# kianmcevoy/audio_analysis

Measured on AMD Instinct MI355X. Metric: IRs/sec full report (STFT+RT60bands+zplane), 48 kHz 10 s IR, higher is better.
Workload: dtype f64; 1 GPU; metrics-only full report on 256 mono synthetic IRs per GPU per step, 10 s @ 48 kHz (SURVEY.md 8d generator), H2D included: every step uploads its batch from pinned host memory (float32, 492 MB) on a copy stream under the previous step's kernels; 4 distinct batches rotate; batch_per_gpu=256, parallelism=file-sharded dp1, gather=final

## Files before the change

### audio_analysis_amd/csrc/ira_stft4.hip

```cpp
#include <cmath>
#include <cstdlib>

#include "ira_fft_reg.h"
#include "ira_log.h"
#include "ira_stft.h"

namespace {

using ira::brev_bits;
using ira::cplx;
using ira::dft_dif;
using ira::powers16;

typedef cplx<double> cdd;

constexpr int M4 = 4096, F4 = M4 + 1, TL4 = 128;
constexpr int ROW4 = 129;
constexpr int E2N4 = 256;
constexpr int EXC4 = 16 * ROW4;
static_assert(EXC4 >= 8 * E2N4 && EXC4 * 2 >= M4, "exchange buffer too small");

__device__ __forceinline__ float db_of4(double re, double im, double floor_pow, float floor_db,
                                        const ira::LogTabEntry* tab) {
  const double p = fma(re, re, im * im);
  if (!(p > floor_pow)) return floor_db;
  return (float)(3.0102999566398120 * ira::log2_table<4>(p, tab));
}

__device__ __forceinline__ double lin_of4(double re, double im, double floor_pow, float floor_db, double floor_lin32,
                                          const ira::LogTabEntry* tab) {
  const double p = fma(re, re, im * im);
  if (!(p > floor_pow)) return floor_lin32;
  const double db = 3.0102999566398120 * ira::log2_table<4>(p, tab);
  const double t = ((double)(float)db - db) * 0.11512925464970228;
  const double y0 = __builtin_amdgcn_rsq(p);
  double g = p * y0;
  const double h = 0.5 * y0;
  const double r = fma(-h, g, 0.5);
  g = fma(g, r, g);
  return g * fma(t, fma(t, 0.5, 1.0), 1.0);
}

constexpr int TL5 = 256;
constexpr int KF5 = 8;

struct __attribute__((aligned(4))) fpair5 { float a, b; };
struct __attribute__((aligned(8))) dpair5 { double a, b; };

__global__ __launch_bounds__(TL5) __attribute__((amdgpu_waves_per_eu(4, 4))) void stft5_kernel(
    const float* __restrict__ x, const int64_t* __restrict__ off, const int32_t* __restrict__ nframes, int hop,
    const double* __restrict__ window, const cdd* __restrict__ tw, double floor_lin, float floor_db,
    float* __restrict__ out, const int64_t* __restrict__ out_off, const int32_t* __restrict__ frame_sel,
    const int64_t* __restrict__ sel_off, int lb_nbins, int lb_kbase, const int32_t* __restrict__ lb_first,
    const int32_t* __restrict__ lb_count, int kfr, int ablate) {
  __shared__ __attribute__((aligned(16))) cdd ex[EXC4];
  __shared__ double wave_energy[2][TL5 / 64];
  __shared__ ira::LogTabEntry ltab[ira::LOGTAB_N];
  __shared__ int lb_range[2];
  __shared__ int frame_bad;
  unsigned bx, by;
  ira::xcd_remap(bx, by);
  const int seg = (int)by;
  const int col0 = (int)bx * kfr;
  const int T_out = ira::uniform(nframes[seg]);
  if (col0 >= T_out) return;
  const int col1 = T_out - col0 < kfr ? T_out : col0 + kfr;
  int q = threadIdx.x;
  double* exd = reinterpret_cast<double*>(ex);
  ira::build_log_table(ltab, q);
  if (q < 2) lb_range[q] = q == 0 ? F4 : 0;

  const float* xs = x + ira::uniform(off[seg]);
  float* os = out + ira::uniform(out_off[seg]);
  const int32_t* fsel = frame_sel ? frame_sel + ira::uniform(sel_off[seg]) : nullptr;
  const double floor_pow = floor_lin * floor_lin;
  const float qnan32 = __uint_as_float(0x7fc00000u);
  int k_lo = 0, k_hi = 0;
  double floor_lin32 = 0.0;
  __syncthreads();
  if (lb_nbins > 0) {
    int lo = F4, hi = 0;
    for (int bb = q; bb < lb_nbins; bb += TL5) {
      const int c = lb_count[bb];
      if (c > 0) {
        const int f0 = lb_kbase + lb_first[bb];
        lo = f0 < lo ? f0 : lo;
        hi = f0 + c > hi ? f0 + c : hi;
      }
    }
    atomicMin(&lb_range[0], lo);
    atomicMax(&lb_range[1], hi);
    __syncthreads();
    k_lo = ira::uniform(lb_range[0]);
    k_hi = ira::uniform(lb_range[1]);
    floor_lin32 = ira::uniform(exp10((double)floor_db * 0.05));
  }

  for (int col = col0; col < col1; ++col) {
    asm volatile("" : "+v"(q));
    const int k1l = q & 15, n3l = q >> 4;
    const bool lower = q < TL4;
    const int64_t frame = fsel ? (int64_t)ira::uniform(fsel[col]) : (int64_t)col;
    const float* fx = xs + frame * hop;
    int u0 = 0;
    asm volatile("" : "+s"(u0));
    cdd wuni[8];
#pragma unroll
    for (int i = 0; i < 8; ++i) wuni[i] = tw[TL5 * i + u0];

    cdd v[16];
    double energy = 0.0;
    {
      float xa[16], xb[16];
      double wa[16], wb[16];
#pragma unroll
      for (int n1 = 0; n1 < 16; ++n1) {
        const int n = n1 * 256 + q;
        if (IRA_ABL(ablate & 2)) { xa[n1] = (float)(n & 7) * 0.125f; xb[n1] = (float)(q & 3); }
        else { const fpair5 p = *reinterpret_cast<const fpair5*>(fx + 2 * n); xa[n1] = p.a; xb[n1] = p.b; }
        if (IRA_ABL(ablate & 1)) { wa[n1] = 0.5 + 1e-4 * n1; wb[n1] = 0.25; }
        else { const dpair5 w = *reinterpret_cast<const dpair5*>(window + 2 * n); wa[n1] = w.a; wb[n1] = w.b; }
      }
      __builtin_amdgcn_sched_barrier(0);
#pragma unroll
      for (int n1 = 0; n1 < 16; ++n1) {
        v[n1] = {(double)xa[n1] * wa[n1], (double)xb[n1] * wb[n1]};
        energy = fma(v[n1].re, v[n1].re, energy);
        energy = fma(v[n1].im, v[n1].im, energy);
      }
    }

    double* we = wave_energy[col & 1];
    {
      const double wsum = ira::wave_sum(energy);
      if ((q & 63) == 0) we[q >> 6] = wsum;
    }
    __syncthreads();
    const double frame_energy = ira::uniform((we[0] + we[1]) + (we[2] + we[3]));
    const bool quiet = !IRA_ABL(ablate & 256) && frame_energy * (4.0 * (2 * M4)) <= floor_pow;

    bool bad_frame = false;
    if (quiet) {
      if (lb_nbins <= 0) {
        float* fo = os + (int64_t)col * F4;
#pragma unroll
        for (int i = 0; i < 8; ++i) {
          const int k = q + TL5 * i;
          fo[k] = floor_db;
          fo[M4 - k] = floor_db;
        }
        if (q == 0) fo[M4 / 2] = floor_db;
        continue;
      }
      double fl = floor_lin32;
      asm volatile("" : "+s"(fl));
#pragma unroll
      for (int i = 0; i < 8; ++i) {
        const int k = q + TL5 * i;
        if (k >= k_lo && k < k_hi) exd[k] = fl;
        if ((M4 - k) >= k_lo && (M4 - k) < k_hi) exd[M4 - k] = fl;
      }
      if (q == 0 && M4 / 2 >= k_lo && M4 / 2 < k_hi) exd[M4 / 2] = fl;
    } else {
      dft_dif<double, 16>(v);
      ira::twiddle16<double, true>(v, tw[2 * q]);

      cdd b[16];
      if (lower) {
#pragma unroll
        for (int k1 = 0; k1 < 16; ++k1) ex[k1 * ROW4 + q] = v[brev_bits(k1, 4)];
      }
      __syncthreads();
#pragma unroll
      for (int n2 = 0; n2 < 8; ++n2) b[n2] = ex[k1l * ROW4 + n2 * 16 + n3l];
      __syncthreads();
      if (!lower) {
#pragma unroll
        for (int k1 = 0; k1 < 16; ++k1) ex[k1 * ROW4 + (q - TL4)] = v[brev_bits(k1, 4)];
      }
      __syncthreads();
#pragma unroll
      for (int n2 = 0; n2 < 8; ++n2) b[8 + n2] = ex[k1l * ROW4 + n2 * 16 + n3l];
      __syncthreads();

      dft_dif<double, 16>(b);
      ira::twiddle16<double, true>(b, tw[32 * n3l]);
      if (lower) {
#pragma unroll
        for (int k2 = 0; k2 < 16; ++k2) ex[k1l + 16 * k2 + E2N4 * n3l] = b[brev_bits(k2, 4)];
      }
      __syncthreads();
#pragma unroll
      for (int n3 = 0; n3 < 8; ++n3) v[n3] = ex[q + E2N4 * n3];
      __syncthreads();
      if (!lower) {
#pragma unroll
        for (int k2 = 0; k2 < 16; ++k2) ex[k1l + 16 * k2 + E2N4 * (n3l - 8)] = b[brev_bits(k2, 4)];
      }
      __syncthreads();
#pragma unroll
      for (int n3 = 0; n3 < 8; ++n3) v[8 + n3] = ex[q + E2N4 * n3];
      __syncthreads();

      dft_dif<double, 16>(v);

      double zkr[8], zpr[8], zki[8], zpi[8], midr, midi;
#pragma unroll
      for (int j = 0; j < 8; ++j) ex[j * TL5 + q] = v[brev_bits(8 + j, 4)];
      __syncthreads();
      {
        const int partner = (TL5 - q) & (TL5 - 1);
#pragma unroll
        for (int i = 0; i < 8; ++i) {
          const int slot = q == 0 ? 8 - i : 7 - i;
          cdd zp = v[0];
          if (!(q == 0 && i == 0)) zp = ex[slot * TL5 + partner];
          zkr[i] = v[brev_bits(i, 4)].re; zki[i] = v[brev_bits(i, 4)].im;
          zpr[i] = zp.re; zpi[i] = zp.im;
        }
      }
      {
        const cdd mid = ex[0];
        midr = mid.re; midi = mid.im;
      }
      if (q == 0) frame_bad = !((zkr[0] - zkr[0]) + (zki[0] - zki[0]) == 0.0) ? 1 : 0;
      __syncthreads();
      bad_frame = frame_bad != 0;

      const cdd wlane = tw[q];
      if (lb_nbins <= 0) {
        float* fo = os + (int64_t)col * F4;
#pragma unroll
        for (int i = 0; i < 8; ++i) {
          const int k = q + TL5 * i;
          const cdd e = {0.5 * (zkr[i] + zpr[i]), 0.5 * (zki[i] - zpi[i])};
          const cdd d = {0.5 * (zkr[i] - zpr[i]), 0.5 * (zki[i] + zpi[i])};
          const cdd o = {d.im, -d.re};
          const cdd wk = ira::cmul(wlane, wuni[i]);
          const cdd pp = ira::cmul(wk, o);
          fo[k] = bad_frame ? qnan32 : db_of4(e.re + pp.re, e.im + pp.im, floor_pow, floor_db, ltab);
          fo[M4 - k] = bad_frame ? qnan32 : db_of4(e.re - pp.re, e.im - pp.im, floor_pow, floor_db, ltab);
        }
        if (q == 0) fo[M4 / 2] = bad_frame ? qnan32 : db_of4(midr, midi, floor_pow, floor_db, ltab);
        continue;
      }
#pragma unroll
      for (int i = 0; i < 8; ++i) {
        const int k = q + TL5 * i;
        const bool need_a = k >= k_lo && k < k_hi, need_b = (M4 - k) >= k_lo && (M4 - k) < k_hi;
        if (!need_a && !need_b) continue;
        const cdd e = {0.5 * (zkr[i] + zpr[i]), 0.5 * (zki[i] - zpi[i])};
        const cdd d = {0.5 * (zkr[i] - zpr[i]), 0.5 * (zki[i] + zpi[i])};
        const cdd o = {d.im, -d.re};
        const cdd wk = ira::cmul(wlane, wuni[i]);
        const cdd pp = ira::cmul(wk, o);
        if (IRA_ABL(ablate & 4)) {
          if (need_a) exd[k] = e.re + pp.re;
          if (need_b) exd[M4 - k] = e.im - pp.im;
          continue;
        }
        if (need_a) exd[k] = lin_of4(e.re + pp.re, e.im + pp.im, floor_pow, floor_db, floor_lin32, ltab);
        if (need_b) exd[M4 - k] = lin_of4(e.re - pp.re, e.im - pp.im, floor_pow, floor_db, floor_lin32, ltab);
      }
      if (q == 0 && M4 / 2 >= k_lo && M4 / 2 < k_hi) exd[M4 / 2] = lin_of4(midr, midi, floor_pow, floor_db, floor_lin32, ltab);
    }
    __syncthreads();
    for (int bb = q; bb < lb_nbins; bb += TL5) {
      const int c = lb_count[bb];
      float val = qnan32;
      if (c > 0) {
        const double* r = exd + lb_kbase + lb_first[bb];
        double acc = r[0];
        for (int k0 = 1; k0 < c; k0 += 8) {
          double v8[8];
#pragma unroll
          for (int u = 0; u < 8; ++u) v8[u] = (k0 + u < c) ? r[k0 + u] : 0.0;
#pragma unroll
          for (int u = 0; u < 8; ++u)
            if (k0 + u < c) acc += v8[u];
        }
        val = (float)(6.0205999132796239 * ira::log2_table<6>(fmax(acc / (double)c, 1e-30), ltab));
      }
      os[(int64_t)bb * T_out + col] = (bad_frame && c > 0) ? qnan32 : val;
    }
    __syncthreads();
  }
}

}

int32_t ira_stft5_launch(const float* x, const int64_t* off, const int32_t* nframes, int32_t nseg, int32_t max_frames,
                         int32_t hop, const void* window, const void* tw, double floor_db, float* out,
                         const int64_t* out_off, const int32_t* frame_sel, const int64_t* sel_off, int32_t lb_nbins,
                         int32_t lb_kbase, const int32_t* lb_first, const int32_t* lb_count, hipStream_t st) {
  const double floor_lin = std::pow(10.0, floor_db / 20.0);
  int kfr = ira_tune_int("IRA_STFT5_K", KF5);
  if (kfr < 1) kfr = 1;
  dim3 grid((max_frames + kfr - 1) / kfr, nseg);
  stft5_kernel<<<grid, TL5, (size_t)ira_tune_int("IRA_STFT5_LDS_PAD", 0), st>>>(x, off, nframes, hop, static_cast<const double*>(window),
                                     static_cast<const cdd*>(tw), floor_lin, (float)floor_db, out, out_off, frame_sel,
                                     sel_off, lb_nbins, lb_kbase, lb_first, lb_count, kfr, ira_tune_int("IRA_STFT5_ABLATE", 0));
  IRA_RETURN_LAUNCH();
}
```

Measured before the change: 16610 IRs/s.

## Skip whole quiet STFT frame chunks via block-level energy bound

Before the per-frame loop, each block sums the squared input over the span covering all of its frames. It bounds the windowed energy by the peak squared window value, and when the bound is below the floor it writes floor values for every frame and exits early. Quiet frames inside the loop also write cached log-bin floor values straight to output instead of filling LDS and taking the shared reduction path. This adds a cheap pre-pass and extra LDS per block. The bound must be conservative or non-quiet frames could be wrongly floored, which matters most for the decaying tails of IRs.

```diff
diff --git a/audio_analysis_amd/csrc/ira_stft4.hip b/audio_analysis_amd/csrc/ira_stft4.hip
--- a/audio_analysis_amd/csrc/ira_stft4.hip
+++ b/audio_analysis_amd/csrc/ira_stft4.hip
@@ -41,11 +41,27 @@
   return g * fma(t, fma(t, 0.5, 1.0), 1.0);
 }
 
+template <bool CONST>
+__device__ __forceinline__ float logbin_mean_db(const double* r, double cst, int c, const ira::LogTabEntry* tab) {
+  double acc = CONST ? cst : r[0];
+  for (int k0 = 1; k0 < c; k0 += 8) {
+    double v8[8];
+#pragma unroll
+    for (int u = 0; u < 8; ++u) v8[u] = (k0 + u < c) ? (CONST ? cst : r[k0 + u]) : 0.0;
+#pragma unroll
+    for (int u = 0; u < 8; ++u)
+      if (k0 + u < c) acc += v8[u];
+  }
+  return (float)(6.0205999132796239 * ira::log2_table<6>(fmax(acc / (double)c, 1e-30), tab));
+}
+
 constexpr int TL5 = 256;
 constexpr int KF5 = 8;
 
 struct __attribute__((aligned(4))) fpair5 { float a, b; };
 struct __attribute__((aligned(8))) dpair5 { double a, b; };
+typedef float fquad5 __attribute__((ext_vector_type(4), aligned(4)));
+constexpr int64_t SPAN5_MAX = 2 * (2 * M4);
 
 __global__ __launch_bounds__(TL5) __attribute__((amdgpu_waves_per_eu(4, 4))) void stft5_kernel(
     const float* __restrict__ x, const int64_t* __restrict__ off, const int32_t* __restrict__ nframes, int hop,
@@ -55,6 +71,9 @@
     const int32_t* __restrict__ lb_count, int kfr, int ablate) {
   __shared__ __attribute__((aligned(16))) cdd ex[EXC4];
   __shared__ double wave_energy[2][TL5 / 64];
+  __shared__ double chunk_energy[TL5 / 64];
+  __shared__ unsigned long long chunk_wmax[TL5 / 64];
+  __shared__ float quiet_val[TL5];
   __shared__ ira::LogTabEntry ltab[ira::LOGTAB_N];
   __shared__ int lb_range[2];
   __shared__ int frame_bad;
@@ -95,6 +114,79 @@
     k_hi = ira::uniform(lb_range[1]);
     floor_lin32 = ira::uniform(exp10((double)floor_db * 0.05));
   }
+  auto quiet_bin = [&](int bb, double fl) -> float {
+    const int c = lb_count[bb];
+    return c > 0 ? logbin_mean_db<true>(nullptr, fl, c, ltab) : qnan32;
+  };
+
+  if (!IRA_ABL(ablate & (256 | 512)) && fsel == nullptr && (int64_t)(col1 - col0 - 1) * hop + 2 * M4 <= SPAN5_MAX) {
+    const int nfr = col1 - col0;
+    const int span = (nfr - 1) * hop + 2 * M4;
+    const float* cx = xs + (int64_t)col0 * hop;
+    const int n4 = span >> 2;
+    double s = 0.0;
+    for (int i0 = 0; i0 < n4; i0 += 4 * TL5) {
+      fquad5 p[4];
+#pragma unroll
+      for (int u = 0; u < 4; ++u) {
+        const int i = i0 + u * TL5 + q;
+        p[u] = i < n4 ? *reinterpret_cast<const fquad5*>(cx + 4 * i) : fquad5{0.0f, 0.0f, 0.0f, 0.0f};
+      }
+#pragma unroll
+      for (int u = 0; u < 4; ++u) {
+        s = fma((double)p[u].x, (double)p[u].x, s);
+        s = fma((double)p[u].y, (double)p[u].y, s);
+        s = fma((double)p[u].z, (double)p[u].z, s);
+        s = fma((double)p[u].w, (double)p[u].w, s);
+      }
+    }
+    if (q < (span & 3)) {
+      const double t = (double)cx[4 * n4 + q];
+      s = fma(t, t, s);
+    }
+    {
+      const double wsum = ira::wave_sum(s);
+      if ((q & 63) == 0) chunk_energy[q >> 6] = wsum;
+    }
+    __syncthreads();
+    const double scaled = ira::uniform((chunk_energy[0] + chunk_energy[1]) + (chunk_energy[2] + chunk_energy[3])) * (4.0 * (2 * M4));
+    if (scaled <= 16.0 * floor_pow) {
+      unsigned long long wb = 0;
+#pragma unroll
+      for (int j = 0; j < 2 * M4 / (2 * TL5); ++j) {
+        const dpair5 w = *reinterpret_cast<const dpair5*>(window + 2 * (j * TL5 + q));
+        const unsigned long long ba = (unsigned long long)__double_as_longlong(w.a * w.a) & 0x7fffffffffffffffull;
+        const unsigned long long bb = (unsigned long long)__double_as_longlong(w.b * w.b) & 0x7fffffffffffffffull;
+        wb = ba > wb ? ba : wb;
+        wb = bb > wb ? bb : wb;
+      }
+#pragma unroll
+      for (int o = 32; o > 0; o >>= 1) {
+        const unsigned long long other = __shfl_xor(wb, o, 64);
+        wb = other > wb ? other : wb;
+      }
+      if ((q & 63) == 0) chunk_wmax[q >> 6] = wb;
+      __syncthreads();
+      unsigned long long wm = chunk_wmax[0];
+#pragma unroll
+      for (int i = 1; i < TL5 / 64; ++i) wm = chunk_wmax[i] > wm ? chunk_wmax[i] : wm;
+      const double wmax2 = ira::uniform(__longlong_as_double((long long)wm));
+      if (scaled * wmax2 <= floor_pow) {
+        if (lb_nbins <= 0) {
+          float* fo = os + (int64_t)col0 * F4;
+          for (int i = q; i < nfr * F4; i += TL5) fo[i] = floor_db;
+        } else {
+          for (int bb = q; bb < lb_nbins; bb += TL5) {
+            const float val = quiet_bin(bb, floor_lin32);
+            float* o = os + (int64_t)bb * T_out + col0;
+            for (int j = 0; j < nfr; ++j) o[j] = val;
+          }
+        }
+        return;
+      }
+    }
+  }
+  bool quiet_built = false;
 
   for (int col = col0; col < col1; ++col) {
     asm volatile("" : "+v"(q));
@@ -154,6 +246,14 @@
       }
       double fl = floor_lin32;
       asm volatile("" : "+s"(fl));
+      if (!IRA_ABL(ablate & 1024)) {
+        if (!quiet_built) {
+          if (q < lb_nbins) quiet_val[q] = quiet_bin(q, fl);
+          quiet_built = true;
+        }
+        for (int bb = q; bb < lb_nbins; bb += TL5) os[(int64_t)bb * T_out + col] = bb < TL5 ? quiet_val[bb] : quiet_bin(bb, fl);
+        continue;
+      }
 #pragma unroll
       for (int i = 0; i < 8; ++i) {
         const int k = q + TL5 * i;
@@ -268,19 +368,7 @@
     for (int bb = q; bb < lb_nbins; bb += TL5) {
       const int c = lb_count[bb];
       float val = qnan32;
-      if (c > 0) {
-        const double* r = exd + lb_kbase + lb_first[bb];
-        double acc = r[0];
-        for (int k0 = 1; k0 < c; k0 += 8) {
-          double v8[8];
-#pragma unroll
-          for (int u = 0; u < 8; ++u) v8[u] = (k0 + u < c) ? r[k0 + u] : 0.0;
-#pragma unroll
-          for (int u = 0; u < 8; ++u)
-            if (k0 + u < c) acc += v8[u];
-        }
-        val = (float)(6.0205999132796239 * ira::log2_table<6>(fmax(acc / (double)c, 1e-30), ltab));
-      }
+      if (c > 0) val = logbin_mean_db<false>(exd + lb_kbase + lb_first[bb], 0.0, c, ltab);
       os[(int64_t)bb * T_out + col] = (bad_frame && c > 0) ? qnan32 : val;
     }
     __syncthreads();
```

Result: faster. 17350 IRs/s, median of 6 (+4.4%).
